# biaslab/GaussianProcessNode

Hardware: AMD Instinct MI355X
Metric: VMP iterations/sec (sparse-GP node sweep, kin40k-shaped synthetic) (higher is better)
Workload: dtype f64

## Files before the change

gaussianprocessnode_amd/csrc/sgp_api.hip:

```cpp
#include "../../include/sgp_hip.h"
#include "sgp_kernels.hip.h"
#include "point_scratch.h"

#include <algorithm>
#include <atomic>
#include <chrono>
#include <cmath>
#include <cstdio>
#include <cstdlib>
#include <dlfcn.h>
#include <cstring>
#include <limits>
#include <mutex>
#include <string>
#include <type_traits>
#include <vector>

using namespace sgp;

namespace {

thread_local std::string g_create_error;
std::atomic<int> g_live_handles{0};

std::mutex g_registry_mutex;
std::vector<sgp_handle*>& registry() { static std::vector<sgp_handle*>* r = new std::vector<sgp_handle*>(); return *r; }
bool g_atexit_registered = false;
void destroy_live_handles_at_exit() {
    std::vector<sgp_handle*> live;
    {
        std::lock_guard<std::mutex> lock(g_registry_mutex);
        live = registry();
    }
    for (sgp_handle* h : live) sgp_destroy(h);
}
void register_handle(sgp_handle* h) {
    std::lock_guard<std::mutex> lock(g_registry_mutex);
    registry().push_back(h);
    if (!g_atexit_registered) {
        g_atexit_registered = true;
        atexit(destroy_live_handles_at_exit);
    }
}
bool unregister_handle(sgp_handle* h) {
    std::lock_guard<std::mutex> lock(g_registry_mutex);
    auto& r = registry();
    auto it = std::find(r.begin(), r.end(), h);
    if (it == r.end()) return false;
    r.erase(it);
    return true;
}

}

enum { WORD_JOIN = 0,
       WORD_DONE = 1,
       WORD_GATE = 2,
       WORD_GRAD = 3,
       WORD_ASM0 = 4,
       WORD_GROUP0 = 8,
       WORD_COUNT = 8 + LAM_MAX_GROUPS };
constexpr int RESERVED_CUS_PER_SE = 2;

struct StatGroup {
    int c0, c1;
    int row_lo, nrows;
    int ntiles;
    SyrkGeom geom;
    int form_step;
    bool masked;
    size_t slab_off;
};

struct SweepPlan {
    hipStream_t stream = nullptr;
    bool overlapped = false;
    bool pack = false;
    bool events = false;
    bool join_word = false;
    bool kuu_interleaved = false;
    bool resident = false;
};

struct StatsRecord {
    double sigma2 = 0.0, jitter = 0.0, inv_ell[MAXD] = {0};
    int32_t family = SGP_KERNEL_SE;
    uint64_t data_gen = ~0ull;
    double w0 = 1.0;
    bool qv = false;
    bool reusable = false;
    bool checked = false;
    bool targets = false;
    bool exact_psi = false;
};
enum : unsigned { STATS_REUSE = 1u, STATS_QV = 2u };

struct sgp_handle {
    sgp_config cfg{};
    int M = 0, Mp = 0, D = 0, dout = 1, Q = 0, Qp = 0, T = 0, TQ = 0;
    int64_t n = 0, n_max = 0;
    double n_nodes = 0;
    bool has_omega = false, has_yv = false, have_data = false, have_kernel = false, have_inducing = false;
    int prior_form = 2;
    bool swept_local = false, swept = false;
    bool in_flight = false;
    bool sync_reported = false;
    hipStream_t last_stream = nullptr;
    uint64_t data_gen = 0;
    int32_t family = SGP_KERNEL_SE;
    int n_ell = 1;
    double *dXu = nullptr, *dXus = nullptr, *dX = nullptr, *dYw = nullptr, *dY = nullptr, *dYv = nullptr, *dOmega = nullptr;
    double *dKuf = nullptr, *dBpart = nullptr, *dSlabs = nullptr, *dStatsOwn = nullptr, *dStats = nullptr, *dDataScal = nullptr;
    double *dKuu = nullptr, *dWk = nullptr, *dKinv = nullptr;
    double *dLam = nullptr, *dWl = nullptr, *dSigma = nullptr, *dR = nullptr, *dXi = nullptr, *dMu = nullptr;
    double *dLambda0 = nullptr, *dXi0 = nullptr, *dOut = nullptr, *dWishart = nullptr, *dTrace = nullptr, *dTmp = nullptr;
    double *dPa = nullptr, *dPb = nullptr, *dKmu = nullptr, *dUvT = nullptr, *dScratch = nullptr, *dOut2 = nullptr, *dUvWork = nullptr;
    double *dGradM = nullptr, *dGradPart = nullptr, *dGrad = nullptr;
    double* dThetaMulti = nullptr;
    double* dSaccK = nullptr;
    long long gate_epoch = 0;
    int spin_limit = JOIN_SPIN_LIMIT;
    double* dCall = nullptr;
    size_t call_capacity = 0;
    int* dInfo = nullptr;
    int64_t* dStamps = nullptr;
    int64_t* dStampTotals = nullptr;
    Params* hParams = nullptr;
    double* hMirror = nullptr;
    long long mirror_epoch = -1;
    double* hStage = nullptr;
    size_t stage_doubles = 0;
    uint64_t params_gen = 1;
    uint64_t main_prep_gen = 0;
    Params* dParams = nullptr;
    Params* dParamsK = nullptr;
    long long* dJoin = nullptr;
    long long join_epoch = 0;
    SweepPlan plan;
    bool gate_side = false;
    long long grad_epoch = 0;
    long long done_epoch = 0;
    const Params* params_src = nullptr;
    double *dTrainX = nullptr, *dTrainY = nullptr;
    int64_t train_N = 0;
    TrainState* dTrain = nullptr;
    Params* dTrainParams = nullptr;
    bool training = false;
    bool train_probit = false;
    double* dXusK = nullptr;
    hipStream_t own = nullptr, side = nullptr;
    hipEvent_t evSide = nullptr, evDone = nullptr;
    hipEvent_t evGroup[LAM_MAX_GROUPS] = {nullptr};
    hipStream_t statM = nullptr;
    int stat_cus_masked = 0;
    bool overlap = false;
    int ngroups = 0;
    StatGroup grp[LAM_MAX_GROUPS];
    long long stat_epoch = 0;
    int env_overlap = -1;
    bool env_interleave = true;
    bool env_no_zero_copy = false;
    int64_t env_predict_chunk = 0;
    bool posterior_set = false;
    bool syrk_wide = false;
    std::vector<int> env_overlap_cols;
    int nblk = 0, ntiles = 0, num_cus = 256;
    SyrkGeom geom{};
    int64_t stats_count = 0;
    size_t slab_capacity = 0;
    double* dBred = nullptr;
    double* dPack = nullptr;
    int64_t pack_count = 0;
    sgp_allreduce_fn allreduce = nullptr;
    void* allreduce_ctx = nullptr;
    void* rccl_comm = nullptr;
    double ryy_data[MAXO * MAXO] = {0};
    StatsRecord stats;
    int32_t last_kind = SGP_SWEEP_FULL;
    std::string err;
};

template <class F>
static void by_family(int32_t family, F&& f) {
    switch (family) {
        case SGP_KERNEL_MATERN12: f(std::integral_constant<int, SGP_KERNEL_MATERN12>{}); break;
        case SGP_KERNEL_MATERN32: f(std::integral_constant<int, SGP_KERNEL_MATERN32>{}); break;
        case SGP_KERNEL_MATERN52: f(std::integral_constant<int, SGP_KERNEL_MATERN52>{}); break;
        default: f(std::integral_constant<int, SGP_KERNEL_SE>{}); break;
    }
}
template <class F>
static void by_dout(int dout, F&& f) {
    switch (dout) {
        case 2: f(std::integral_constant<int, 2>{}); break;
        case 3: f(std::integral_constant<int, 3>{}); break;
        default: f(std::integral_constant<int, 4>{}); break;
    }
}

static const double* omega_of(const sgp_handle* h) { return h->has_omega ? h->dOmega : nullptr; }

static void stats_formed(sgp_handle* h) {
    const Params& P = *h->hParams;
    StatsRecord& r = h->stats;
    r.sigma2 = P.sigma2; r.jitter = P.jitter; r.family = h->family; r.data_gen = h->data_gen; r.w0 = P.W[0];
    for (int d = 0; d < MAXD; ++d) r.inv_ell[d] = P.inv_ell[d];
    r.qv = h->swept_local = true;
}
static void stats_reusable(sgp_handle* h) { h->stats.reusable = true; h->stats.checked = h->stats.targets = false; }
static void stats_drop(sgp_handle* h, unsigned what) {
    if (what & STATS_REUSE) h->stats.reusable = false;
    if (what & STATS_QV) h->stats.qv = false;
}
static void stats_targets(sgp_handle* h, bool pending) { h->stats.targets = pending; }
static void stats_checked(sgp_handle* h, bool ok) { if (ok) h->stats.checked = true; else h->stats.reusable = false; }
static void stats_exact_psi(sgp_handle* h, bool on) { h->stats.exact_psi = on; }
static bool kernel_matches(const sgp_handle* h) {
// ... 247 lines not shown
#define ALLOC(ptr, count)                                            \
    do {                                                             \
        hipError_t e_ = dalloc(&(ptr), (count));                     \
        if (e_ != hipSuccess) {                                      \
            g_create_error = std::string("hipMalloc failed for " #ptr ": ") + hipGetErrorString(e_); \
            sgp_destroy(h);                                          \
            return SGP_ERR_NOMEM;                                    \
        }                                                            \
    } while (0)
    ALLOC(h->dXu, (size_t)h->M * h->D);
    ALLOC(h->dXus, Mp * h->D);
    ALLOC(h->dX, nmax * h->D);
    ALLOC(h->dYw, nmax * h->dout);
    ALLOC(h->dY, nmax * h->dout);
    ALLOC(h->dYv, nmax);
    ALLOC(h->dOmega, nmax);
    ALLOC(h->dKuf, Mp * nmax);
    ALLOC(h->dBpart, nblk_max * h->dout * Mp);
    ALLOC(h->dBred, (size_t)h->T * h->dout * 4 * TB);
    ALLOC(h->dSlabs, h->slab_capacity);
    ALLOC(h->dStatsOwn, (size_t)h->stats_count);
    ALLOC(h->dJoin, WORD_COUNT);
    ALLOC(h->dDataScal, SGP_S_COUNT + (size_t)h->dout * h->dout);
    ALLOC(h->dKuu, Mp * Mp);
    ALLOC(h->dWk, Mp * Mp);
    ALLOC(h->dKinv, Mp * Mp);
    ALLOC(h->dSaccK, Mp * Mp);
    ALLOC(h->dLam, Qp * Qp);
    ALLOC(h->dWl, Qp * Qp);
    ALLOC(h->dSigma, Qp * Qp);
    ALLOC(h->dR, Qp * Qp);
    ALLOC(h->dTmp, Qp * Qp);
    ALLOC(h->dUvT, Qp * Qp);
    ALLOC(h->dScratch, 3 * POTRF_SCRATCH);
    hipMemset(h->dScratch, 0, sizeof(double) * 3 * POTRF_SCRATCH);
    ALLOC(h->dOut2, SGP_R_COUNT);
    ALLOC(h->dUvWork, (2 + 2 * (size_t)h->TQ) * Qp);
    ALLOC(h->dLambda0, Qp * Qp);
    ALLOC(h->dXi, Qp);
    ALLOC(h->dMu, Qp);
    ALLOC(h->dXi0, Qp);
    ALLOC(h->dOut, SGP_R_COUNT);
    ALLOC(h->dWishart, MAXO * MAXO);
    ALLOC(h->dTrace, (size_t)TRACE_BLOCKS + std::max((size_t)TRACE_BLOCKS * MAXO * MAXO, (size_t)h->TQ * (h->TQ + 1) * 4));
    ALLOC(h->dInfo, 4);
    ALLOC(h->dStamps, STAMP_STRIDE * SGP_T_COUNT);
    ALLOC(h->dStampTotals, SGP_T_COUNT + 1 + 2 * SGP_T_COUNT);
    ALLOC(h->dParams, 1);
    ALLOC(h->dParamsK, 1);
    ALLOC(h->dXusK, Mp * h->D);
    {
        if (const char* lim = getenv("SGP_SPIN_LIMIT")) h->spin_limit = std::max(1, atoi(lim));
        if (const char* ov = getenv("SGP_OVERLAP")) h->env_overlap = atoi(ov);
        if (const char* zc = getenv("SGP_NO_ZERO_COPY")) h->env_no_zero_copy = atoi(zc) != 0;
        if (const char* ni = getenv("SGP_INTERLEAVE")) h->env_interleave = atoi(ni) != 0;
        if (const char* pc = getenv("SGP_PREDICT_CHUNK")) h->env_predict_chunk = std::max(1LL, atoll(pc));
        if (const char* oc = getenv("SGP_OVERLAP_COLS"))
            for (const char* q = oc; *q;) {
                h->env_overlap_cols.push_back(atoi(q));
                while (*q && *q != ',') ++q;
                if (*q == ',') ++q;
            }
    }
    if (cfg->flags & SGP_FLAG_KEEP_KUF) {
        ALLOC(h->dPa, (4 * (size_t)h->T + 4) * nmax);
        h->dPb = h->dPa + 2 * (size_t)h->T * nmax;
        h->dKmu = h->dPb + 2 * (size_t)h->T * nmax;
    }
#undef ALLOC
    h->dStats = h->dStatsOwn;
    if (hipHostMalloc(reinterpret_cast<void**>(&h->hParams), sizeof(Params), hipHostMallocDefault) != hipSuccess) {
        g_create_error = "hipHostMalloc failed for the parameter block";
        sgp_destroy(h);
        return SGP_ERR_NOMEM;
    }
    {
        const size_t per_point = (size_t)h->D + 2 * (size_t)h->dout + 2;
        h->stage_doubles = std::min<size_t>((size_t)h->n_max * per_point, (size_t)1 << 19) + SGP_S_COUNT + (size_t)h->dout * h->dout;
        if (hipHostMalloc(reinterpret_cast<void**>(&h->hStage), sizeof(double) * h->stage_doubles, hipHostMallocDefault) != hipSuccess) {
            h->hStage = nullptr;
            h->stage_doubles = 0;
            (void)hipGetLastError();
        }
    }
    if (hipHostMalloc(reinterpret_cast<void**>(&h->hMirror), sizeof(double) * (SGP_R_COUNT + 2), hipHostMallocDefault) != hipSuccess) {
        h->hMirror = nullptr;
        (void)hipGetLastError();
    } else {
        for (int i = 0; i < SGP_R_COUNT + 2; ++i) h->hMirror[i] = -1.0;
    }
    memset(h->hParams, 0, sizeof(Params));
    h->hParams->sigma2 = 1.0;
    for (int d = 0; d < MAXD; ++d) h->hParams->inv_ell[d] = 1.0;
    h->hParams->W[0] = 1.0;
    h->hParams->prior_iso = 1.0;
    h->params_src = h->hParams;
    if (hipStreamCreateWithFlags(&h->own, hipStreamNonBlocking) != hipSuccess ||
        create_low_priority_stream(&h->side) != hipSuccess ||
        hipEventCreateWithFlags(&h->evSide, hipEventDisableTiming) != hipSuccess ||
        hipEventCreateWithFlags(&h->evDone, hipEventDisableTiming) != hipSuccess) {
        g_create_error = "stream/event creation failed";
        sgp_destroy(h);
        return SGP_ERR_HIP;
    }
    for (int g = 0; g < LAM_MAX_GROUPS; ++g)
        if (hipEventCreateWithFlags(&h->evGroup[g], hipEventDisableTiming) != hipSuccess) {
// ... 18 lines not shown
    hipMemset(h->dStamps, 0, STAMP_STRIDE * SGP_T_COUNT * sizeof(int64_t));
    hipMemset(h->dStampTotals, 0, (SGP_T_COUNT + 1 + 2 * SGP_T_COUNT) * sizeof(int64_t));
    hipMemset(h->dMu, 0, Qp * sizeof(double));
    hipMemset(h->dXi0, 0, Qp * sizeof(double));
    *out = h;
    return 0;
}

extern "C" int sgp_destroy(sgp_handle* h) {
    if (!h) return 0;
    if (!unregister_handle(h)) return 0;
    h->allreduce = nullptr;
    h->allreduce_ctx = nullptr;
    if (hipSetDevice(h->cfg.device) != hipSuccess || hipDeviceSynchronize() != hipSuccess) {
        (void)hipGetLastError();
        --g_live_handles;
        delete h;
        return 0;
    }
    void* bufs[] = {h->dXu, h->dXus, h->dX, h->dYw, h->dY, h->dYv, h->dOmega, h->dKuf, h->dBpart, h->dSlabs, h->dStatsOwn,
                    h->dDataScal, h->dKuu, h->dWk, h->dKinv, h->dLam, h->dWl, h->dSigma, h->dR, h->dTmp, h->dLambda0,
                    h->dXi, h->dMu, h->dXi0, h->dOut, h->dWishart, h->dTrace, h->dInfo, h->dStamps, h->dParams, h->dPa,
                    h->dUvT, h->dScratch, h->dParamsK, h->dXusK, h->dOut2, h->dStampTotals, h->dUvWork,
                    h->dGradM, h->dGradPart, h->dGrad, h->dCall, h->dSaccK, h->dThetaMulti,
                    h->dTrainX, h->dTrainY, h->dTrain, h->dTrainParams, h->dJoin, h->dPack, h->dBred};
    for (void* b : bufs) if (b) hipFree(b);
    if (h->hParams) hipHostFree(h->hParams);
    if (h->hStage) hipHostFree(h->hStage);
    if (h->hMirror) hipHostFree(h->hMirror);
    if (h->evSide) hipEventDestroy(h->evSide);
    if (h->evDone) hipEventDestroy(h->evDone);
    for (hipEvent_t e : h->evGroup) if (e) hipEventDestroy(e);
    if (h->own) hipStreamDestroy(h->own);
    if (h->side) hipStreamDestroy(h->side);
    if (h->statM) hipStreamDestroy(h->statM);
    --g_live_handles;
    delete h;
    return 0;
}

extern "C" int sgp_set_inducing(sgp_handle* h, const double* Xu) {
    if (!h || !Xu) return fail(h, SGP_ERR_ARG, "sgp_set_inducing: null argument");
    if (int qrc = quiesce(h)) return qrc;
    h->data_gen++;
    stats_drop(h, STATS_REUSE);
    HIPCHK(h, hipSetDevice(h->cfg.device));
    HIPCHK(h, hipMemcpy(h->dXu, Xu, sizeof(double) * h->M * h->D, hipMemcpyHostToDevice));
    h->have_inducing = true;
    h->params_gen++;
    h->swept = h->swept_local = false;
    return 0;
}

static double model_overlap_end(const sgp_handle* h, int64_t n, bool wide, const int* cuts, int ncuts, double* classic_end) {
    const int T = h->T;
    auto syrk_us = [&](int row_lo, int nrows, int cus) {
        const SyrkGeom g = syrk_geometry(row_lo, nrows, cus, n, wide);
        return g.wide ? 13.0 + 0.029 * g.chunk : 5.0 + 0.18 * g.chunk;
    };
    const bool dk = wide;
    const double asm0 = dk ? 11.5 : 8.0, asmm = dk ? 5.0 : 11.0, step = 17.0, margin = dk ? 0.0 : 4.0, forming = dk ? 5.0 : 2.5;
    const double mstart = dk ? 8.0 : 2.0, launch = dk ? 5.5 : 0.0;
    if (classic_end) *classic_end = syrk_us(0, T, h->num_cus) - launch + asm0 + step * T;
    double ready[LAM_MAX_COLS];
    double t = syrk_us(T - cuts[0], cuts[0], h->num_cus) - launch + asm0;
    for (int c = 0; c < cuts[0]; ++c) ready[c] = t;
    t -= asm0 - mstart;
    for (int g = 0; g < ncuts; ++g) {
        const int c0 = cuts[g], c1 = (g + 1 < ncuts) ? cuts[g + 1] : T;
        t += syrk_us(T - c1, c1 - c0, h->stat_cus_masked) - launch + asmm;
        for (int c = c0; c < c1; ++c) ready[c] = t;
    }
    double end = ready[0];
    for (int j = 0; j < T; ++j) {
        bool forms = false;
        for (int g = 0; g < ncuts; ++g) forms = forms || cuts[g] == j;
        end = std::max(end, ready[j] + (j >= cuts[0] ? margin : 0.0)) + step + (forms ? forming : 0.0);
    }
    return end;
}

constexpr int64_t GATE_MIN = 10000;

static void plan_overlap(sgp_handle* h, int64_t n) {
    h->overlap = false;
    h->ngroups = 0;
    const int T = h->T;
    const int64_t np = h->allreduce ? h->n_max : n;
    const bool wide = h->allreduce ? np * (int64_t)h->ntiles >= GATE_MIN : h->syrk_wide;
    if (!h->statM || h->env_overlap == 0 || h->dout != 1 || T < 3 || T > LAM_MAX_COLS || h->training || np < 1 ||
        (!wide && h->env_overlap != 1))
        return;
    std::vector<int> cuts;
    for (int c : h->env_overlap_cols) if (c > 0 && c < T && (cuts.empty() || c > cuts.back())) cuts.push_back(c);
    if (cuts.empty()) {
        double classic = 0.0, best = 1e300;
        int cand[2];
        for (int a = 1; a < T; ++a) {
            cand[0] = a; cand[1] = a;
            const double e = model_overlap_end(h, np, wide, cand, 1, &classic);
            if (e < best - 0.3) { best = e; cuts.assign(cand, cand + 1); }
            if (!wide || h->allreduce) continue;
            if (T < 6) continue;
            for (int b = T - 1; b > a; --b) {
                cand[1] = b;
                const double m1 = 13.0 + 0.029 * syrk_geometry(T - b, b - a, h->stat_cus_masked, np, true).chunk;
                const double m2 = 13.0 + 0.029 * syrk_geometry(0, T - b, h->stat_cus_masked, np, true).chunk;
                if (m1 > 45.0 || m2 > 45.0) continue;
                const double e2 = model_overlap_end(h, np, wide, cand, 2, &classic);
                if (e2 < best - 0.3) { best = e2; cuts.assign(cand, cand + 2); }
            }
        }
        if (h->env_overlap != 1 && best > classic - (wide ? 1.0 : 5.0)) return;
    }
    if ((int)cuts.size() + 1 > LAM_MAX_GROUPS) return;
    size_t off = 0;
    int c0 = 0;
    for (size_t g = 0; g <= cuts.size(); ++g) {
        StatGroup& G = h->grp[g];
        G.c0 = c0;
        G.c1 = (g < cuts.size()) ? cuts[g] : T;
        G.row_lo = T - G.c1;
        G.nrows = G.c1 - G.c0;
        G.masked = g > 0;
        G.form_step = G.c0;
        G.geom = syrk_geometry(G.row_lo, G.nrows, G.masked ? h->stat_cus_masked : h->num_cus, n, h->syrk_wide);
        G.ntiles = G.geom.ntiles;
        G.slab_off = off;
        off += syrk_items(G.geom) * TB * TB;
        c0 = G.c1;
    }
    if (off > h->slab_capacity) {
        double* bigger = nullptr;
        if (hipMalloc(reinterpret_cast<void**>(&bigger), sizeof(double) * off) != hipSuccess) { (void)hipGetLastError(); return; }
        hipFree(h->dSlabs);
        h->dSlabs = bigger;
        h->slab_capacity = off;
    }
    h->ngroups = (int)cuts.size() + 1;
    h->overlap = true;
}

static int set_point_count(sgp_handle* h, int64_t n) {
    h->n = n;
    h->nblk = (int)((n + TB - 1) / TB);
    h->gate_side = n * (int64_t)h->ntiles >= GATE_MIN;
    h->syrk_wide = h->gate_side;
    h->geom = syrk_geometry(0, h->T, h->num_cus - (h->gate_side ? 0 : SYRK_RESERVED_CUS), n, h->syrk_wide);
    if (syrk_items(h->geom) * TB * TB > h->slab_capacity)
        return fail(h, SGP_ERR_ARG, "sgp_set_data: internal slab capacity exceeded");
    plan_overlap(h, n);
    return 0;
}

static void form_targets(sgp_handle* h, const double* y_mean, const double* y_var, const double* pt_weight, int64_t n,
                         double n_nodes, std::vector<double>& yw, std::vector<double>& scal) {
    const int dout = h->dout;
    yw.assign((size_t)std::max<int64_t>(n, 1) * dout, 0.0);
    scal.assign(SGP_S_COUNT + (size_t)dout * dout, 0.0);
    double s_w = 0.0;
    for (int64_t i = 0; i < n; ++i) s_w += pt_weight ? pt_weight[i] : 1.0;
    for (int o = 0; o < dout; ++o)
        for (int64_t i = 0; i < n; ++i) yw[(size_t)o * n + i] = y_mean[(size_t)o * n + i] * (pt_weight ? pt_weight[i] : 1.0);
    for (int a = 0; a < dout; ++a)
        for (int b = 0; b < dout; ++b) {
            double s = 0.0;
            for (int64_t i = 0; i < n; ++i) s += yw[(size_t)a * n + i] * y_mean[(size_t)b * n + i];
            scal[SGP_S_COUNT + a + (size_t)b * dout] = s;
        }
    double s_yy = scal[SGP_S_COUNT];
    if (y_var)
        for (int64_t i = 0; i < n; ++i) s_yy += (pt_weight ? pt_weight[i] : 1.0) * y_var[i];
    scal[SGP_S_YY] = s_yy;
    if (dout == 1) scal[SGP_S_COUNT] = s_yy;
    scal[SGP_S_W] = s_w;
    scal[SGP_S_N] = (n_nodes > 0) ? n_nodes : (double)n;
    for (int i = 0; i < dout * dout; ++i) h->ryy_data[i] = scal[SGP_S_COUNT + i];
}
// ... 291 lines not shown
    if (h->n <= 0) { ga = syrk_geometry(0, T, h->num_cus, 0); }
    hipLaunchKernelGGL(k_assemble, dim3(T, T + 1, assemble_z(ga)), dim3(256), 0, s, h->dSlabs, h->dBpart, h->dDataScal,
                       pack ? h->dPack : h->dStats, Mp, T, ga, h->n > 0 ? h->nblk : 0, h->dout,
                       SGP_S_COUNT + h->dout * h->dout, 1, h->dStamps + STAMP_STRIDE * SGP_T_LOCAL, h->dInfo + 1, (long long*)nullptr, 0LL,
                       pack ? 1 : 0, h->dBred, h->has_omega ? 1 : 0);
}

static int exchange_stats(sgp_handle* h, hipStream_t s, int tile0, int ntile, bool with_tail);
static int enqueue_stats_overlapped(sgp_handle* h, const SweepPlan& p) {
    const int Mp = h->Mp, T = h->T;
    hipStream_t own = p.stream;
    const bool sharded = p.pack;
    prep_main(h, own, h->n <= 0);
    if (h->n > 0) launch_gram(h, own, true);
    hipLaunchKernelGGL(k_join_wait, dim3(1), dim3(64), 0, h->statM, (const long long*)(h->dJoin + WORD_ASM0), h->stat_epoch,
                       h->spin_limit, h->dInfo + 3, (int)SYNC_LATE_COLUMN, 8);
    for (int g = 0; g < h->ngroups; ++g) {
        const StatGroup& G = h->grp[g];
        hipStream_t s = G.masked ? h->statM : own;
        if (h->n > 0)
            launch_syrk(G.geom, s, h->dKuf, omega_of(h), h->dSlabs + G.slab_off, Mp, h->n,
                        h->dStamps + STAMP_STRIDE * SGP_T_SYRK, g == 0 ? h->dJoin + WORD_GATE : (long long*)nullptr, h->gate_epoch);
        hipLaunchKernelGGL(k_assemble, dim3(G.nrows, T + (g == 0 ? 1 : 0), assemble_z(G.geom)), dim3(256), 0, s, h->dSlabs + G.slab_off, h->dBpart,
                           h->dDataScal, sharded ? h->dPack : h->dStats, Mp, T, G.geom, h->nblk, h->dout,
                           SGP_S_COUNT + h->dout * h->dout, g == 0 ? 1 : 0, h->dStamps + STAMP_STRIDE * SGP_T_LOCAL,
                           g == 0 ? h->dInfo + 1 : (int*)nullptr, g == 0 ? h->dJoin + WORD_ASM0 : (long long*)nullptr, h->stat_epoch,
                           sharded ? 1 : 0, h->dBred, h->has_omega ? 1 : 0);
        if (sharded) {
            if (int xrc = exchange_stats(h, s, G.geom.tile0, G.geom.ntiles, g == 0)) return xrc;
            if (G.masked && hipEventRecord(h->evGroup[g], s) != hipSuccess) return fail(h, SGP_ERR_HIP, "hipEventRecord failed (statistics group)");
        } else if (G.masked)
            hipLaunchKernelGGL(k_join_set, dim3(1), dim3(64), 0, s, h->dJoin + WORD_GROUP0 + g, h->stat_epoch);
    }
    return 0;
}

static void enqueue_finish1(sgp_handle* h, hipStream_t s, const SweepPlan& p) {
    const int M = h->M, Mp = h->Mp, Q = h->Q, Qp = h->Qp, TQ = h->TQ;
    LamForm form;
    memset(&form, 0, sizeof form);
    form.stats = h->dStats; form.Lambda0 = h->dLambda0; form.xi0 = h->dXi0; form.xi = h->dXi; form.P = h->dParams;
    form.M = M; form.Mp = Mp; form.d_out = h->dout; form.Q = Q; form.prior_form = h->prior_form;
    form.stamps = h->dStamps + STAMP_STRIDE * SGP_T_FINISH1;
    form.spin_limit = h->spin_limit;
    form.sync_status = h->dInfo + 3;
    form.trace_chain = 1;
    hipEvent_t step_wait[LAM_MAX_COLS] = {nullptr};
    bool any_wait = false;
    if (p.overlapped) {
        form.col_words = h->dJoin + WORD_GROUP0;
        form.col_need = h->stat_epoch;
        for (int g = 0; g < h->ngroups; ++g) {
            for (int c = h->grp[g].c0; c < h->grp[g].c1; ++c) {
                form.form_step[c] = (unsigned char)h->grp[g].form_step;
                form.col_group[c] = (h->grp[g].masked && !p.pack && !p.resident) ? (unsigned char)g : (unsigned char)0xff;
            }
            if (h->grp[g].masked && p.pack && !p.resident) { step_wait[h->grp[g].form_step] = h->evGroup[g]; any_wait = true; }
        }
    }
    double* uvt0 = h->dUvWork + 2 * (size_t)Qp;
    PotrfSeq lam(h->dLam, Qp, TQ, h->dInfo + 1, Qp, h->dScratch + POTRF_SCRATCH, s, h->dWl, &form, h->dTmp, h->dXi, uvt0,
                 any_wait ? step_wait : nullptr);
    lam.mu_acc = h->dUvWork;
    lam.uv_part = uvt0 + (size_t)TQ * Qp;
    if (p.kuu_interleaved) {
        PotrfSeq kuu(h->dKuu, h->Mp, h->T, h->dInfo + 0, h->M, h->dScratch, h->side, h->dWk, nullptr, h->dSaccK);
        while (!lam.done() || !kuu.done()) {
            if (!lam.done()) lam.next();
            if (!kuu.done()) kuu.next();
        }
        kuu_tail(h, h->side, p.join_word);
    } else {
        while (!lam.done()) lam.next();
    }
}

static double* mirror_for(const sgp_handle* h) {
    return (h->hMirror && !h->env_no_zero_copy && !h->training) ? h->hMirror : nullptr;
}

static void launch_traces(sgp_handle* h, hipStream_t s, const double* Rv = nullptr) {
    hipLaunchKernelGGL(k_trace_kinv, dim3(TRACE_BLOCKS), dim3(256), 0, s, h->dStats, h->dKinv, h->dTrace, h->M, h->Mp);
    hipLaunchKernelGGL(k_trace_R, dim3(TRACE_BLOCKS), dim3(256), 0, s, h->dStats, Rv ? Rv : h->dR, h->dTrace + TRACE_BLOCKS, h->M, h->Mp, h->dout,
                       h->Qp, (int64_t*)nullptr);
}

static void enqueue_finish2(sgp_handle* h, hipStream_t s, bool join_word) {
    const int M = h->M, Mp = h->Mp, Q = h->Q, Qp = h->Qp, TQ = h->TQ;
    double* uvt = h->dUvWork + 2 * (size_t)Qp;
    double* uvpart = uvt + (size_t)TQ * Qp;
    const int nata = TQ * (TQ + 1) / 2 * 4;
    double* traceR = h->dTrace + TRACE_BLOCKS;
    const double* partK = h->dTrace;
    int nK = TRACE_BLOCKS, nR = TRACE_BLOCKS;
    UvArgs uv;
    uv.Wp = h->dWl; uv.t = uvt; uv.muacc = h->dUvWork; uv.partial = uvpart; uv.LR = h->dUvT;
    uv.stamps = h->dStamps + STAMP_STRIDE * SGP_T_FINISH1;
    uv.join = join_word ? h->dJoin + WORD_JOIN : nullptr;
    uv.join_need = h->join_epoch;
    uv.spin_limit = h->spin_limit;
    uv.sync_status = h->dInfo + 3;
    if (h->dout == 1) {
        launch_ata(h->dWl, h->dSigma, Qp, TQ, s, 1, h->dMu, h->dR, h->dStats, h->dKinv, traceR, &uv, h->dTmp);
        partK = traceR + nata;
        nK = nR = nata;
    } else {
        launch_ata(h->dWl, h->dSigma, Qp, TQ, s, 1, h->dMu, h->dR, nullptr, nullptr, nullptr, &uv, h->dTmp);
        launch_traces(h, s);
    }
    hipLaunchKernelGGL(k_scalars, dim3(1), dim3(256), 0, s, h->dStats, partK, nK, (const double*)traceR, nR, h->dMu, h->dKuu,
// ... 2173 lines not shown
```

gaussianprocessnode_amd/csrc/sgp_kernels.hip.h:

```cpp
#pragma once
#include <hip/hip_runtime.h>
#include <stdint.h>
#include <utility>

namespace sgp {

constexpr int TB = 64;
constexpr int PS = 80;
constexpr int KB = 16;
constexpr int MAXD = 32;
constexpr int MAXO = 4;
constexpr int LT = TB + 1;

typedef double d4 __attribute__((ext_vector_type(4)));

struct Params {
    double sigma2;
    double jitter;
    double E_logw;
    double n_override;
    double inv_ell[MAXD];
    double W[MAXO * MAXO];
    double prior_iso;
    double pad[7];
// ... 1151 lines not shown
    if (wave & 1) {
        const int rb = 16 * wave, cb = 16 * (wave - 1);
        double* Tw = T + (wave >> 1) * (16 * 17);
        d4 acc = (d4){0.0, 0.0, 0.0, 0.0};
#pragma unroll
        for (int s4 = 0; s4 < 4; ++s4)
            acc = __builtin_amdgcn_mfma_f64_16x16x4f64(S[(rb + li) * LT + cb + 4 * s4 + lk],
                                                       Wt[(cb + 4 * s4 + lk) * LT + cb + li], acc, 0, 0, 0);
#pragma unroll
        for (int r = 0; r < 4; ++r) Tw[(lk + 4 * r) * 17 + li] = acc[r];
        __builtin_amdgcn_wave_barrier();
        acc = (d4){0.0, 0.0, 0.0, 0.0};
#pragma unroll
        for (int s4 = 0; s4 < 4; ++s4)
            acc = __builtin_amdgcn_mfma_f64_16x16x4f64(Wt[(rb + li) * LT + rb + 4 * s4 + lk], Tw[(4 * s4 + lk) * 17 + li],
                                                       acc, 0, 0, 0);
#pragma unroll
        for (int r = 0; r < 4; ++r) Wt[(rb + lk + 4 * r) * LT + cb + li] = -acc[r];
    }
    __syncthreads();
    {
        const int ti = wave >> 1, tj = wave & 1;
        d4 acc = (d4){0.0, 0.0, 0.0, 0.0};
#pragma unroll
        for (int s4 = 0; s4 < 8; ++s4)
            acc = __builtin_amdgcn_mfma_f64_16x16x4f64(S[(32 + 16 * ti + li) * LT + 4 * s4 + lk],
                                                       Wt[(4 * s4 + lk) * LT + 16 * tj + li], acc, 0, 0, 0);
#pragma unroll
        for (int r = 0; r < 4; ++r) T[(16 * ti + lk + 4 * r) * 33 + 16 * tj + li] = acc[r];
        __syncthreads();
        acc = (d4){0.0, 0.0, 0.0, 0.0};
#pragma unroll
        for (int s4 = 0; s4 < 8; ++s4)
            acc = __builtin_amdgcn_mfma_f64_16x16x4f64(Wt[(32 + 16 * ti + li) * LT + 32 + 4 * s4 + lk],
                                                       T[(4 * s4 + lk) * 33 + 16 * tj + li], acc, 0, 0, 0);
#pragma unroll
        for (int r = 0; r < 4; ++r) Wt[(32 + 16 * ti + lk + 4 * r) * LT + 16 * tj + li] = -acc[r];
    }
    __syncthreads();
}

struct TileRegs { double v[16]; };
__device__ __forceinline__ void tile_g2r(TileRegs& t, const double* __restrict__ A, size_t ld, int row0, int col0) {
#pragma unroll
    for (int u = 0; u < 8; ++u) {
        const int e = (threadIdx.x & 255) + 256 * u, c = e >> 5, r = (e & 31) * 2;
        const double2 w = *reinterpret_cast<const double2*>(A + (size_t)(col0 + c) * ld + row0 + r);
        t.v[2 * u] = w.x;
        t.v[2 * u + 1] = w.y;
    }
}
constexpr int LAM_MAX_GROUPS = 8;
constexpr int LAM_MAX_COLS = 64;
struct LamForm {
    const double* stats;
    const double* Lambda0;
    const double* xi0;
    double* xi;
    const Params* P;
    int M, Mp, d_out, Q, prior_form;
    int64_t* stamps;
    const long long* col_words;
    long long col_need;
    unsigned char form_step[LAM_MAX_COLS], col_group[LAM_MAX_COLS];
    int spin_limit;
    int* sync_status;
    int trace_chain;
};
__device__ __forceinline__ double load_agent(const double* p) {
    return __hip_atomic_load((const __attribute__((address_space(1))) double*)p, __ATOMIC_RELAXED, __HIP_MEMORY_SCOPE_AGENT);
}
template <bool DENSE, bool MULTI, bool BYPASS = false>
__device__ __forceinline__ double lambda_entry(const LamForm& f, int gi, int gj, int Qp, double prior_iso, double w00) {
    const bool inside = gi < f.Q && gj < f.Q;
    const int si = inside ? gi : 0, sj = inside ? gj : 0;
    int a = 0, i = si, b = 0, j = sj;
    if constexpr (MULTI) { a = si / f.M; i = si % f.M; b = sj / f.M; j = sj % f.M; }
    double psi;
    if constexpr (BYPASS) psi = load_agent(f.stats + (size_t)j * f.Mp + i); else psi = f.stats[(size_t)j * f.Mp + i];
    const double diag = (gi == gj) ? 1.0 : 0.0;
    double prior, w;
    if constexpr (DENSE) prior = f.Lambda0[(size_t)sj * Qp + si]; else prior = diag * prior_iso;
    if constexpr (MULTI) w = f.P->W[a + b * f.d_out]; else w = w00;
    const double m = inside ? 1.0 : 0.0;
    return fma(m * w, psi, fma(m, prior, (1.0 - m) * diag));
}
template <bool DENSE, bool MULTI, bool BYPASS>
__device__ __forceinline__ void tile_form_r_impl(TileRegs& t, const LamForm& f, int Qp, int row0, int col0) {
    const double prior_iso = BYPASS ? load_agent(&f.P->prior_iso) : f.P->prior_iso, w00 = BYPASS ? load_agent(&f.P->W[0]) : f.P->W[0];
#pragma unroll
    for (int u = 0; u < 16; ++u) {
        const int e = (threadIdx.x & 255) + 256 * (u >> 1), c = e >> 5, r = (e & 31) * 2 + (u & 1);
        t.v[u] = lambda_entry<DENSE, MULTI, BYPASS>(f, Qp - 1 - (row0 + r), Qp - 1 - (col0 + c), Qp, prior_iso, w00);
    }
}
__device__ __forceinline__ void tile_form_r(TileRegs& t, const LamForm& f, int Qp, int row0, int col0, bool bypass = false) {
    const bool dense = f.prior_form == 1, multi = f.d_out > 1;
    if (bypass && !multi) {
        if (dense) tile_form_r_impl<true, false, true>(t, f, Qp, row0, col0); else tile_form_r_impl<false, false, true>(t, f, Qp, row0, col0);
        return;
    }
    if (dense) { if (multi) tile_form_r_impl<true, true, false>(t, f, Qp, row0, col0); else tile_form_r_impl<true, false, false>(t, f, Qp, row0, col0); }
    else       { if (multi) tile_form_r_impl<false, true, false>(t, f, Qp, row0, col0); else tile_form_r_impl<false, false, false>(t, f, Qp, row0, col0); }
}
__device__ __forceinline__ void tile_r2s(double* S, const TileRegs& t) {
#pragma unroll
    for (int u = 0; u < 16; ++u) {
        const int e = (threadIdx.x & 255) + 256 * (u >> 1), c = e >> 5, r = (e & 31) * 2 + (u & 1);
        S[r * LT + c] = t.v[u];
    }
}
__device__ __forceinline__ void tile_g2s(double* S, const double* __restrict__ A, size_t ld, int row0, int col0) {
    TileRegs t;
    tile_g2r(t, A, ld, row0, col0);
    tile_r2s(S, t);
}
__device__ __forceinline__ void tile_fetch(TileRegs& t, bool do_form, bool load_old, const double* __restrict__ A, const LamForm& f,
                                           int ld, int row0, int col0, bool bypass) {
    if (do_form) {
        tile_form_r(t, f, ld, row0, col0, bypass);
        if (load_old) {
            TileRegs o;
            tile_g2r(o, A, ld, row0, col0);
#pragma unroll
            for (int u = 0; u < 16; ++u) t.v[u] += o.v[u];
        }
    } else if (load_old) {
        tile_g2r(t, A, ld, row0, col0);
    } else {
#pragma unroll
        for (int u = 0; u < 16; ++u) t.v[u] = 0.0;
    }
}
__device__ __forceinline__ void tile_s2g(const double* S, double* __restrict__ A, size_t ld, int row0, int col0) {
    double2 v[8];
#pragma unroll
    for (int u = 0; u < 8; ++u) {
        const int e = (threadIdx.x & 255) + 256 * u, c = e >> 5, r = (e & 31) * 2;
        v[u] = make_double2(S[r * LT + c], S[(r + 1) * LT + c]);
    }
#pragma unroll
    for (int u = 0; u < 8; ++u) {
        const int e = (threadIdx.x & 255) + 256 * u, c = e >> 5, r = (e & 31) * 2;
        *reinterpret_cast<double2*>(A + (size_t)(col0 + c) * ld + row0 + r) = v[u];
    }
}
__device__ __forceinline__ void tile_s2g_t(const double* S, double* __restrict__ A, size_t ld, int row0, int col0) {
    double2 v[8];
#pragma unroll
    for (int u = 0; u < 8; ++u) {
        const int e = (threadIdx.x & 255) + 256 * u, c = e >> 5, r = (e & 31) * 2;
        v[u] = make_double2(S[c * LT + r], S[c * LT + r + 1]);
    }
#pragma unroll
    for (int u = 0; u < 8; ++u) {
        const int e = (threadIdx.x & 255) + 256 * u, c = e >> 5, r = (e & 31) * 2;
        *reinterpret_cast<double2*>(A + (size_t)(col0 + c) * ld + row0 + r) = v[u];
    }
}
__device__ __forceinline__ void tile_sub_acc(double* S, const Acc4& acc, int lane, int wr, int wc) {
#pragma unroll
    for (int ti = 0; ti < 2; ++ti)
#pragma unroll
        for (int tj = 0; tj < 2; ++tj)
#pragma unroll
            for (int r = 0; r < 4; ++r)
                S[acc_row(lane, wr, ti, r) * LT + acc_col(lane, wc, tj)] -= acc.t[ti][tj][r];
}

constexpr int PS32 = 48;

__device__ __forceinline__ void load_panel32_n(double* panel, const double* __restrict__ G, size_t ld, int row0, int col0, int tid) {
    double2 v0[2], v1[2];
#pragma unroll
    for (int u = 0; u < 2; ++u) {
        int t = tid + 256 * u, k = t >> 3, rq = t & 7;
        const double* src = G + (size_t)(col0 + k) * ld + row0 + rq * 4;
        v0[u] = *reinterpret_cast<const double2*>(src);
        v1[u] = *reinterpret_cast<const double2*>(src + 2);
    }
#pragma unroll
    for (int u = 0; u < 2; ++u) {
        int t = tid + 256 * u, k = t >> 3, rq = t & 7;
        double* dst = panel + k * PS32 + rq * 4;
        dst[0] = v0[u].x; dst[1] = v0[u].y; dst[2] = v1[u].x; dst[3] = v1[u].y;
    }
}
__device__ __forceinline__ void load_panel32_t(double* panel, const double* __restrict__ G, size_t ld, int row0, int col0, int tid) {
    double2 v0[2], v1[2];
#pragma unroll
    for (int u = 0; u < 2; ++u) {
        int t = tid + 256 * u, i = t & 31, g = t >> 5;
        const double* src = G + (size_t)(col0 + i) * ld + row0 + g * 4;
        v0[u] = *reinterpret_cast<const double2*>(src);
        v1[u] = *reinterpret_cast<const double2*>(src + 2);
    }
#pragma unroll
// ... 297 lines not shown
constexpr int POTRF_TWINS = 2;
__host__ __device__ constexpr int potrf_twins(int Tn, int j) { return (Tn - j >= 2) ? POTRF_TWINS : 0; }
constexpr int POTRF_SCRATCH = 3 * TB * TB + 64 + 64;
constexpr int POTRF_LOGDET = 3 * TB * TB + 64;
__global__ void __launch_bounds__(PSTEP_THREADS) k_potrf_step(double* __restrict__ A, int ld, int j, int Tn, int* __restrict__ info,
                                                    int n_valid, double* __restrict__ scratch, double* __restrict__ Winv,
                                                    double* __restrict__ Sacc, const double* __restrict__ tv_xi,
                                                    double* __restrict__ tv_t, double* __restrict__ mu_acc,
                                                    double* __restrict__ uv_part, LamForm form) {
    __shared__ __attribute__((aligned(16))) double lds[2 * TB * PS];
    __shared__ __attribute__((aligned(16))) double tiles[2 * TB * LT];
    __shared__ double dprep[4 * DPB];
    __shared__ double rinv[TB];
    TraceScope trace((form.trace_chain ? 16 : 40) + j);
    const bool xgroup = threadIdx.x >= 256;
    const int tid = threadIdx.x & 255, lane = tid & 63, wave = tid >> 6, wr = wave >> 1, wc = wave & 1;
    {
        const int npot = (Tn - j) * (Tn - j + 1) / 2 + potrf_twins(Tn, j);
        if ((int)blockIdx.x >= npot) {
            int e = blockIdx.x - npot;
            const int nfin = (j >= 2) ? 2 * (j - 1) : 0;
            const int npre = (j < Tn) ? nfin : 0;
            const int nsig = (Sacc && j >= 2 && j < Tn) ? (j - 1) * j / 2 : 0;
            if (e == nfin + npre + nsig) { tvec_role<8>(A, Winv, tv_xi, tv_t, ld, j - 1, lds); return; }
            if (e > nfin + npre + nsig) { mu_row_tile(Winv, tv_t, mu_acc, uv_part, ld, Tn, j - 2, e - (nfin + npre + nsig) - 1, lds); return; }
            if (xgroup) return;
            if (e < nfin) winv_row_tile(A, Winv, ld, j - 1, e >> 1, e & 1, lds, 2, tiles);
            else if (e < nfin + npre) { e -= nfin; winv_row_tile(A, Winv, ld, j, e >> 1, e & 1, lds, 1); }
            else if (e < nfin + npre + nsig) {
                int I, J;
                tile_from_index(e - nfin - npre, I, J);
                sigma_row_tile(Winv, Sacc, ld, j - 2, I, J, lds, tiles);
            }
            return;
        }
    }
    int a, b, tw = 0;
    {
        const int nown = (Tn - j) * (Tn - j + 1) / 2;
        if ((int)blockIdx.x >= nown) { a = 1; b = 0; tw = blockIdx.x - nown + 1; }
        else tile_from_index(blockIdx.x, a, b);
    }
    const int i0 = (j + a) * TB, k0 = (j + b) * TB, j0 = j * TB;
    double* P0 = lds;
    double* P1 = lds + TB * PS;
    double* S = tiles;
    double* X = tiles + TB * LT;
    Acc4 accX;
    acc_zero(accX);
    const bool panel = (b == 0);
    const bool diag_inv = panel && a == 0 && Winv != nullptr;
    if (xgroup && !(panel && (a != 0 || diag_inv))) return;
    const bool lam = form.stats != nullptr;
    const int fstep = lam ? (int)form.form_step[j + b] : -1;
    const bool do_form = lam && fstep == j;
    const bool load_old = !lam || fstep < j || j >= 2;
    const bool xi_duty = lam && j == 0 && blockIdx.x == gridDim.x - 1;
    if (!lam && j == 0 && !panel) return;
    bool bypass = false;
    if (lam && form.col_words) {
        if (xi_duty && form.col_group[0] != 0xff) bypass = wait_stat_group(form, form.col_group[0]);
        if (do_form && form.col_group[j + b] != 0xff) bypass = wait_stat_group(form, form.col_group[j + b]) || bypass;
        if (j == 0 && !do_form) {
            if (xi_duty) form_xi(form, ld, tid, bypass);
            return;
        }
        if (blockIdx.x == 0 && !xgroup) trace_mark(200 + j);
    }
    double* Dn_out = scratch + (size_t)(1 + (j & 1)) * TB * TB;
    const double* Dn_in = scratch + (size_t)(2 - (j & 1)) * TB * TB;
    auto move_prev = [&]() {
        const int q0 = (j - 1) * TB;
        for (int e = tid; e < TB * TB; e += 256) A[(size_t)(q0 + (e >> 6)) * ld + q0 + (e & 63)] = scratch[e];
    };
    TileRegs rX, rS, rD;
    if (lam && j == 0) stamp_enter(form.stamps);
    STEP_TRACE(0);
    if (panel) {
        long long* tw_words = reinterpret_cast<long long*>(scratch + 3 * TB * TB);
        if (!xgroup) {
            if (a != 0 || diag_inv) __builtin_amdgcn_s_setprio(3);
            tile_fetch(rS, do_form, load_old, A, form, ld, j0, j0, bypass);
            if (j > 0) {
                tile_g2r(rD, Dn_in, TB, 0, 0);
#pragma unroll
                for (int u = 0; u < 16; ++u) rS.v[u] -= rD.v[u];
            }
            if (xi_duty) form_xi(form, ld, tid, bypass);
            if (a == 0 && tid == 0) tw_words[(j + 1) & 1] = 0;
            tile_r2s(S, rS);
            STEP_TRACE(1);
            __syncthreads();
            STEP_TRACE(2);
            if (a == 0 && j > 0 && !diag_inv) move_prev();
            const bool has_solve = (a != 0) || diag_inv;
            const int ntwf = 1 + potrf_twins(Tn, j);
            int fcount = 0, fR[3], fC[3];
            d4 fg[3];
#pragma unroll
            for (int q = 0; q < 3; ++q) {
                fg[q] = (d4){0.0, 0.0, 0.0, 0.0};
                fR[q] = fC[q] = 0;
                const int t = tw + ntwf * ((wave - 1) + 2 * q);
                if (a == 1 && (wave == 1 || wave == 2) && t < 10) { tile_from_index(t, fR[q], fC[q]); fcount = q + 1; }
            }
            auto fsyrk = [&](int c) {
#pragma unroll
                for (int q = 0; q < 3; ++q)
                    if (q < fcount) syrk_slice(fg[q], X, fR[q], fC[q], c);
// ... 63 lines not shown
                            accX.t[1][0] = __builtin_amdgcn_mfma_f64_16x16x4f64(a1, b0, accX.t[1][0], 0, 0, 0);
                            accX.t[1][1] = __builtin_amdgcn_mfma_f64_16x16x4f64(a1, b1, accX.t[1][1], 0, 0, 0);
                            ap += 4 * PS; bp += 4 * PS;
                        }
                    }
                    if (done == 4) { tile_sub_acc(X, accX, lane, wr, wc); done = 5; }
                }
                STEP_TRACE(3 + 2 * it);
                __syncthreads();
                STEP_TRACE(4 + 2 * it);
            }
        }
        const bool next = (a == 1);
        const int tw_need = (next && tw == 0) ? potrf_twins(Tn, j) : 0;
        bool tw_ready = true;
#pragma unroll 1
        for (int it = 0; it < 4; ++it) {
            if (it == 3 && tw_need > 0 && lane == 0) tw_ready = join_ready(tw_words + (j & 1), tw_need);
            const bool off = (wave == 2 && it == 0) || (wave == 3 && (it == 1 || it == 2));
            if (!off) trsm_interval(X, S, dprep, rinv, wave, it);
            STEP_TRACE(13 + 2 * it);
            __syncthreads();
            STEP_TRACE(14 + 2 * it);
        }
        STEP_TRACE(11);
        if (!below) tile_s2g_t(X, Winv, ld, j0, j0);
        else if (tw == 0) {
            if (tw_need > 0 && lane == 0 && !tw_ready) {
                int it = 0;
                while (!join_ready(tw_words + (j & 1), tw_need)) {
                    if (++it >= (1 << 21)) { atomicMin(info, -1); break; }
                    __builtin_amdgcn_s_sleep(16);
                }
            }
            tile_s2g(X, A, ld, i0, j0);
        }
        STEP_TRACE(12);
        return;
    }
    tile_fetch(rX, do_form, load_old, A, form, ld, i0, k0, bypass);
    if (xi_duty) form_xi(form, ld, tid, bypass);
    if (j > 0) {
        const int p0 = (j - 1) * TB;
        load_panel_n(P0, A, ld, i0, p0, TB, tid);
        if (a != b) load_panel_n(P1, A, ld, k0, p0, TB, tid);
        __syncthreads();
        tile_mma(accX, P0, (a != b) ? P1 : P0, TB, lane, wr, wc);
        __syncthreads();
    }
    tile_r2s(X, rX);
    __syncthreads();
    tile_sub_acc(X, accX, lane, wr, wc);
    __syncthreads();
    tile_s2g(X, A, ld, i0, k0);
}

__device__ __forceinline__ void load_v_column(double (&v)[64], const double* __restrict__ Wp, int Qp, int kb, int j) {
    const double2* src = reinterpret_cast<const double2*>(Wp + (size_t)(Qp - 1 - j) * Qp + (Qp - 64 * (kb + 1)));
#pragma unroll
    for (int u = 0; u < 32; ++u) {
        const double2 w = src[u];
        v[63 - 2 * u] = w.x;
        v[62 - 2 * u] = w.y;
    }
}

struct UvArgs {
    const double* Wp;
    const double* t;
    const double* muacc;
    const double* partial;
    double* LR;
    int64_t* stamps;
    const long long* join;
    long long join_need;
    int spin_limit;
    int* sync_status;
};
__global__ void k_join_wait(const long long* w, long long need, int spin_limit, int* sync_status, int bit, int trace_slot) {
    TraceScope trace(trace_slot);
    if (threadIdx.x == 0 && blockIdx.x == 0) spin_until(w, need, spin_limit, sync_status, bit);
}
__global__ void k_join_set(long long* w, long long v) {
    if (threadIdx.x == 0 && blockIdx.x == 0)
        __hip_atomic_store((__attribute__((address_space(1))) long long*)w, v, __ATOMIC_RELAXED, __HIP_MEMORY_SCOPE_AGENT);
}
__device__ __forceinline__ void uv_cols_role(const UvArgs& u, int Qp, int kb, int jb) {
    const int lane = threadIdx.x, j = 64 * jb + lane;
    double* out = u.LR + (size_t)(64 * kb) * Qp + j;
    if (kb > jb) {
#pragma unroll 16
        for (int kk = 0; kk < 64; ++kk) out[(size_t)kk * Qp] = 0.0;
        stamp_exit(u.stamps);
        return;
    }
    double v[64];
    load_v_column(v, u.Wp, Qp, kb, j);
    double T = 0.0;
    for (int b0 = jb; b0 > kb; b0 -= 8) {
        double pv[8];
#pragma unroll
        for (int e = 0; e < 8; ++e) {
            const int b = b0 - e;
            pv[e] = u.partial[(size_t)max(b, kb + 1) * Qp + j] * ((b > kb) ? 1.0 : 0.0);
        }
#pragma unroll
// ... 2612 lines not shown
```

Baseline: 4728.

## Form late stat-group columns early inside the preceding Cholesky step

Adds an 'early form' mode for overlapped stat groups. The step before a group's form step runs the trailing update first, then waits on the group's stats, forms the Lambda tile and adds it into the updated tile before storing. This moves the wait on the masked SYRK off the critical path of the next step. The planner's cost model now tracks early forming per group and also searches three-cut splits when T is at least 8. It adds kernel branching and an extra wait inside the tile epilogue, and it relies on the cost model's constants being right.

```diff
diff --git a/gaussianprocessnode_amd/csrc/sgp_api.hip b/gaussianprocessnode_amd/csrc/sgp_api.hip
--- a/gaussianprocessnode_amd/csrc/sgp_api.hip
+++ b/gaussianprocessnode_amd/csrc/sgp_api.hip
@@ -68,6 +68,7 @@
     int ntiles;
     SyrkGeom geom;
     int form_step;
+    bool early;
     bool masked;
     size_t slab_off;
 };
@@ -163,6 +164,7 @@
     int64_t env_predict_chunk = 0;
     bool posterior_set = false;
     bool syrk_wide = false;
+    int env_early_form = -1;
     std::vector<int> env_overlap_cols;
     int nblk = 0, ntiles = 0, num_cus = 256;
     SyrkGeom geom{};
@@ -516,6 +518,7 @@
     {
         if (const char* lim = getenv("SGP_SPIN_LIMIT")) h->spin_limit = std::max(1, atoi(lim));
         if (const char* ov = getenv("SGP_OVERLAP")) h->env_overlap = atoi(ov);
+        if (const char* ef = getenv("SGP_EARLY_FORM")) h->env_early_form = atoi(ef) != 0;
         if (const char* zc = getenv("SGP_NO_ZERO_COPY")) h->env_no_zero_copy = atoi(zc) != 0;
         if (const char* ni = getenv("SGP_INTERLEAVE")) h->env_interleave = atoi(ni) != 0;
         if (const char* pc = getenv("SGP_PREDICT_CHUNK")) h->env_predict_chunk = std::max(1LL, atoll(pc));
@@ -640,7 +643,8 @@
     return 0;
 }
 
-static double model_overlap_end(const sgp_handle* h, int64_t n, bool wide, const int* cuts, int ncuts, double* classic_end) {
+static double model_overlap_end(const sgp_handle* h, int64_t n, bool wide, const int* cuts, int ncuts, double* classic_end,
+                                bool* early_out = nullptr) {
     const int T = h->T;
     auto syrk_us = [&](int row_lo, int nrows, int cus) {
         const SyrkGeom g = syrk_geometry(row_lo, nrows, cus, n, wide);
@@ -659,12 +663,23 @@
         t += syrk_us(T - c1, c1 - c0, h->stat_cus_masked) - launch + asmm;
         for (int c = c0; c < c1; ++c) ready[c] = t;
     }
+    const double lead = 6.0, add = 2.5;
+    bool early[LAM_MAX_COLS] = {false};
     double end = ready[0];
     for (int j = 0; j < T; ++j) {
+        double start = end;
         bool forms = false;
-        for (int g = 0; g < ncuts; ++g) forms = forms || cuts[g] == j;
-        end = std::max(end, ready[j] + (j >= cuts[0] ? margin : 0.0)) + step + (forms ? forming : 0.0);
-    }
+        for (int g = 0; g < ncuts && g < LAM_MAX_COLS; ++g)
+            if (cuts[g] == j && !early[g]) { start = std::max(start, ready[j] + margin); forms = true; }
+        end = start + step + (forms ? forming : 0.0);
+        for (int g = 0; g < ncuts && g < LAM_MAX_COLS; ++g)
+            if (cuts[g] == j + 1) {
+                early[g] = h->env_early_form >= 0 ? h->env_early_form != 0 : ready[j + 1] + margin <= start + lead;
+                if (early[g]) end = std::max(end, std::max(start + lead, ready[j + 1] + margin) + add);
+            }
+    }
+    if (early_out)
+        for (int g = 0; g < ncuts && g < LAM_MAX_COLS; ++g) early_out[g] = early[g];
     return end;
 }
 
@@ -683,7 +698,7 @@
     for (int c : h->env_overlap_cols) if (c > 0 && c < T && (cuts.empty() || c > cuts.back())) cuts.push_back(c);
     if (cuts.empty()) {
         double classic = 0.0, best = 1e300;
-        int cand[2];
+        int cand[3];
         for (int a = 1; a < T; ++a) {
             cand[0] = a; cand[1] = a;
             const double e = model_overlap_end(h, np, wide, cand, 1, &classic);
@@ -697,11 +712,22 @@
                 if (m1 > 45.0 || m2 > 45.0) continue;
                 const double e2 = model_overlap_end(h, np, wide, cand, 2, &classic);
                 if (e2 < best - 0.3) { best = e2; cuts.assign(cand, cand + 2); }
+                if (T < 8) continue;
+                for (int c = T - 1; c > b; --c) {
+                    cand[2] = c;
+                    const double n2 = 13.0 + 0.029 * syrk_geometry(T - c, c - b, h->stat_cus_masked, np, true).chunk;
+                    const double n3 = 13.0 + 0.029 * syrk_geometry(0, T - c, h->stat_cus_masked, np, true).chunk;
+                    if (n2 > 45.0 || n3 > 45.0) continue;
+                    const double e3 = model_overlap_end(h, np, wide, cand, 3, &classic);
+                    if (e3 < best - 0.3) { best = e3; cuts.assign(cand, cand + 3); }
+                }
             }
         }
         if (h->env_overlap != 1 && best > classic - (wide ? 1.0 : 5.0)) return;
     }
     if ((int)cuts.size() + 1 > LAM_MAX_GROUPS) return;
+    bool early[LAM_MAX_COLS] = {false};
+    (void)model_overlap_end(h, np, wide, cuts.data(), (int)cuts.size(), nullptr, early);
     size_t off = 0;
     int c0 = 0;
     for (size_t g = 0; g <= cuts.size(); ++g) {
@@ -712,6 +738,7 @@
         G.nrows = G.c1 - G.c0;
         G.masked = g > 0;
         G.form_step = G.c0;
+        G.early = g > 0 && early[g - 1];
         G.geom = syrk_geometry(G.row_lo, G.nrows, G.masked ? h->stat_cus_masked : h->num_cus, n, h->syrk_wide);
         G.ntiles = G.geom.ntiles;
         G.slab_off = off;
@@ -1109,10 +1136,10 @@
         form.col_need = h->stat_epoch;
         for (int g = 0; g < h->ngroups; ++g) {
             for (int c = h->grp[g].c0; c < h->grp[g].c1; ++c) {
-                form.form_step[c] = (unsigned char)h->grp[g].form_step;
+                form.form_step[c] = (unsigned char)(h->grp[g].form_step | (h->grp[g].early ? LAM_FORM_EARLY : 0));
                 form.col_group[c] = (h->grp[g].masked && !p.pack && !p.resident) ? (unsigned char)g : (unsigned char)0xff;
             }
-            if (h->grp[g].masked && p.pack && !p.resident) { step_wait[h->grp[g].form_step] = h->evGroup[g]; any_wait = true; }
+            if (h->grp[g].masked && p.pack && !p.resident) { step_wait[h->grp[g].form_step - (h->grp[g].early ? 1 : 0)] = h->evGroup[g]; any_wait = true; }
         }
     }
     double* uvt0 = h->dUvWork + 2 * (size_t)Qp;
diff --git a/gaussianprocessnode_amd/csrc/sgp_kernels.hip.h b/gaussianprocessnode_amd/csrc/sgp_kernels.hip.h
--- a/gaussianprocessnode_amd/csrc/sgp_kernels.hip.h
+++ b/gaussianprocessnode_amd/csrc/sgp_kernels.hip.h
@@ -1227,6 +1227,7 @@
 }
 constexpr int LAM_MAX_GROUPS = 8;
 constexpr int LAM_MAX_COLS = 64;
+constexpr int LAM_FORM_EARLY = 0x80;
 struct LamForm {
     const double* stats;
     const double* Lambda0;
@@ -1318,6 +1319,14 @@
     for (int u = 0; u < 8; ++u) {
         const int e = (threadIdx.x & 255) + 256 * u, c = e >> 5, r = (e & 31) * 2;
         *reinterpret_cast<double2*>(A + (size_t)(col0 + c) * ld + row0 + r) = v[u];
+    }
+}
+__device__ __forceinline__ void tile_s2g_add(const double* S, const TileRegs& t, double* __restrict__ A, size_t ld, int row0, int col0) {
+#pragma unroll
+    for (int u = 0; u < 8; ++u) {
+        const int e = (threadIdx.x & 255) + 256 * u, c = e >> 5, r = (e & 31) * 2;
+        *reinterpret_cast<double2*>(A + (size_t)(col0 + c) * ld + row0 + r) =
+            make_double2(S[r * LT + c] + t.v[2 * u], S[(r + 1) * LT + c] + t.v[2 * u + 1]);
     }
 }
 __device__ __forceinline__ void tile_s2g_t(const double* S, double* __restrict__ A, size_t ld, int row0, int col0) {
@@ -1721,9 +1730,12 @@
     const bool diag_inv = panel && a == 0 && Winv != nullptr;
     if (xgroup && !(panel && (a != 0 || diag_inv))) return;
     const bool lam = form.stats != nullptr;
-    const int fstep = lam ? (int)form.form_step[j + b] : -1;
-    const bool do_form = lam && fstep == j;
-    const bool load_old = !lam || fstep < j || j >= 2;
+    const int fword = lam ? (int)form.form_step[j + b] : 0;
+    const int fstep = lam ? (fword & (LAM_FORM_EARLY - 1)) : -1;
+    const bool early = (fword & LAM_FORM_EARLY) != 0;
+    const bool do_form = lam && (early ? (j == 0 && fstep == 1) : fstep == j);
+    const bool late_form = lam && early && j >= 1 && fstep == j + 1;
+    const bool load_old = !lam || j >= 2 || (early ? (j == 1 && fstep == 1) : fstep < j);
     const bool xi_duty = lam && j == 0 && blockIdx.x == gridDim.x - 1;
     if (!lam && j == 0 && !panel) return;
     bool bypass = false;
@@ -1893,6 +1905,13 @@
     __syncthreads();
     tile_sub_acc(X, accX, lane, wr, wc);
     __syncthreads();
+    if (late_form) {
+        bool late = false;
+        if (form.col_words && form.col_group[j + b] != 0xff) late = wait_stat_group(form, form.col_group[j + b]);
+        tile_form_r(rX, form, ld, i0, k0, late);
+        tile_s2g_add(X, rX, A, ld, i0, k0);
+        return;
+    }
     tile_s2g(X, A, ld, i0, k0);
 }
 
```

After: 4778, median of 6. +1.1%, better.
